# hammershock/3dgs-avatar-release

Measured on AMD Instinct MI355X. Metric: render fps (fwd+bwd) @200k Gaussians 1024x1024 SH3, higher is better.
Workload: dtype f32; 1 GPU; config3: 200k Gaussians, 1024x1024, SH deg 3, forward+backward; shs+scales+rotations inputs, L1 loss (L1 fused into the rasterizer: l1_target); tile_rect=1, l1=fused, long_lists=0, gaussians=200000, width=1024, height=1024, sh_degree=3, frames_per_rank=1857, total_frames=1857, ranks=1, backend=none, parallelism=frames sharded x1

## Files before the change

3dgs-avatar-release_amd/csrc/binning.hip:

```cpp
#include "common.h"

__global__ __launch_bounds__(256) void first_pair_kernel(const uint32_t* __restrict__ tiles,
                                                         const uint32_t* __restrict__ wave_tiles, float* __restrict__ rec,
                                                         int P, unsigned long long* __restrict__ count,
                                                         unsigned long long* host_count) {
    __shared__ unsigned long long wb[4];
    const int tid = threadIdx.x, lane = tid & 63, wid = tid >> 6;
    const int w0 = 4 * (int)blockIdx.x;
    unsigned long long before = 0;
    for (int w = tid; w < w0; w += 256) before += wave_tiles[w];
#pragma unroll
    for (int d = 32; d >= 1; d >>= 1) before += __shfl_xor(before, d, 64);
    if (lane == 0) wb[wid] = before;
    const int i = blockIdx.x * 256 + tid;
    const uint32_t v = i < P ? tiles[i] : 0u;
    uint32_t x = v;
#pragma unroll
    for (int d = 1; d < 64; d <<= 1) {
        const uint32_t y = __shfl_up(x, d, 64);
        if (lane >= d) x += y;
    }
    __syncthreads();
    const unsigned long long block_base = (wb[0] + wb[1]) + (wb[2] + wb[3]);
    uint32_t woff = 0;
// ... 395 lines not shown
                                                          const uint32_t* __restrict__ keys, int mode, int ntiles,
                                                          uint32_t* __restrict__ order, const PairCount pc,
                                                          const FillJob fill, const LongLists ll) {
    if (blockIdx.x > 0) {
        if (fill.clean && *fill.clean == MARKS_CLEAN) return;
        const uint4 ones = make_uint4(0xFFFFFFFFu, 0xFFFFFFFFu, 0xFFFFFFFFu, 0xFFFFFFFFu);
        for (size_t k = (size_t)(blockIdx.x - 1) * 1024 + threadIdx.x; k < fill.quads; k += (size_t)(gridDim.x - 1) * 1024)
            if (fill.stream) store_stream(&fill.ptr[k], ones); else fill.ptr[k] = ones;
        return;
    }
    __shared__ uint32_t hist[1024];
    __shared__ uint32_t wmax[16];
    __shared__ uint32_t wsum[16];
    if (mode < 0) return;
    tile_order_body<HELD>(ranges, keys, mode, ntiles, order, pc, ll, hist, wmax, wsum);
}

#define BM_LD 33
#ifndef TW_STOP_AFTER
#define TW_STOP_AFTER 99
#endif
template <bool CW>
__global__ __launch_bounds__(TBK_THREADS) void tile_write_kernel(const uint4* __restrict__ ranklist,
                                                                 const uint32_t* __restrict__ seg_start, int P, int gx,
                                                                 int gy, int nbx, int nblocks, int nseg, int ntiles,
                                                                 const uint32_t* __restrict__ seg_cnt,
                                                                 const uint32_t* __restrict__ tile_tot,
                                                                 uint2* __restrict__ ranges, uint32_t* __restrict__ order,
                                                                 uint32_t* __restrict__ point_list, const PairCount pc,
                                                                 const LongLists ll) {
// ... 197 lines not shown

int launch_tile_order(const uint32_t* ranges, const uint32_t* keys, int mode, int ntiles, uint32_t* order, PairCount pc,
                      FillJob fill, LongLists ll, int debug, hipStream_t s) {
    const size_t pieces = (fill.quads + 1023) / 1024;
    const int side = fill.ptr ? (int)(pieces < 255 ? pieces : 255) : 0;
    if (ntiles <= 32 * 1024)
        hipLaunchKernelGGL(tile_order_kernel<true>, dim3(1 + side), dim3(1024), 0, s, reinterpret_cast<const uint2*>(ranges),
                           keys, mode, ntiles, order, pc, fill, ll);
    else
        hipLaunchKernelGGL(tile_order_kernel<false>, dim3(1 + side), dim3(1024), 0, s, reinterpret_cast<const uint2*>(ranges),
                           keys, mode, ntiles, order, pc, fill, ll);
    GS_LAUNCH_CHECK("tile_order", debug, s);
    return GS_OK;
}

int launch_tile_lists(const uint4* ranklist, const uint32_t* chunk_pairs, uint32_t* seg_start, int P, int gx, int gy, TileCounts tc, uint32_t* ranges,
                      uint32_t* order, uint32_t* point_list, PairCount pc, LongLists ll, bool totals_zeroed, int debug,
                      hipStream_t s) {
    uint32_t* seg_cnt = tc.seg_cnt;
    const BinGrid G = bin_grid(gx, gy);
    const int nseg = bin_segments(G, P);
    const int ntiles = gx * gy;
    if (!totals_zeroed) {
        const int zrc = gs_zero_async(tc.tile_tot, tc.zero_bytes, "tile_totals.zero", s);
        if (zrc != GS_OK) return zrc;
    }
    {
        int band_rows = TC_CELLS / (gx + 1) - 1;
        if (band_rows < 1) return GS_E_TOO_LARGE;
        if (band_rows > gy) band_rows = gy;
// ... 21 lines not shown
```

3dgs-avatar-release_amd/csrc/capi.hip:

```cpp
#include "common.h"
#include "boundary.h"
#include "sorted_lists.h"
#include <string.h>
#include <stdlib.h>
#include <atomic>
#include <chrono>
#include <mutex>
#include <vector>

static thread_local int g_last_hip = 0;
static thread_local const char* g_last_stage = "";
void gs_set_error(int hip_err, const char* stage) {
    g_last_hip = hip_err;
    g_last_stage = stage;
}

struct TuneSwitch {
    const char* name;
    int key, def;
    const char* env;
    bool (*ok)(int);
};
static const TuneSwitch k_tune[GS_TUNE_COUNT] = {
    {"xcd_map", GS_TUNE_XCD_MAP, 1, nullptr, nullptr},
    {"depth_sort", GS_TUNE_DEPTH_SORT, 1, nullptr, nullptr},
    {"nt_stores", GS_TUNE_NT_STORES, 1, nullptr, nullptr},
    {"bwd_chunks", GS_TUNE_BWD_CHUNKS, 1, nullptr, nullptr},
    {"fwd4", GS_TUNE_FWD4, 1, "GSPLAT_FWD4", nullptr},
    {"small_tiles", GS_TUNE_SMALL_TILES, BWD_CHUNK_MAX_TILES, nullptr, nullptr},
    {"shared_qlist", GS_TUNE_SHARED_QLIST, 1, nullptr, nullptr},
    {"ones_fast", GS_TUNE_ONES_FAST, 1, nullptr, nullptr},
    {"bwd_order", GS_TUNE_BWD_ORDER, 1, nullptr, nullptr},
    {"fwd_marks", GS_TUNE_FWD_MARKS, 1, nullptr, nullptr},
    {"fwdc_ch", GS_TUNE_FWDC_CH, (int)FWDC_CH_MIN, "GSPLAT_FWDC_CH", [](int v) { return v >= 64 && (v & (v - 1)) == 0; }},
    {"fwdc_div", GS_TUNE_FWDC_DIV, (int)FWD4_TOTAL_DIV, "GSPLAT_FWDC_DIV", [](int v) { return v >= 1; }},
};
struct TuneState {
    std::atomic<int> v[GS_TUNE_COUNT];
    TuneState() {
        for (const TuneSwitch& t : k_tune) {
            int value = t.def;
            if (const char* e = t.env ? getenv(t.env) : nullptr) {
                const int x = atoi(e);
                if (!t.ok || t.ok(x)) value = x;
            }
            v[t.key].store(value);
        }
    }
};
static TuneState& tune_state() {
// ... 136 lines not shown
    ql.ckpt = ql.chunks > 1 ? writable(im.ckpt) : nullptr;
    ql.ck_start = ql.chunks > 1 ? writable(im.ck_start) : nullptr;
    return ql;
}
template <bool RO>
static void quad_lists_chunked(QuadLists& ql, const ImgView& own, const ImgViewT<RO>& list) {
    ql.chunked = 1;
    ql.cw_hdr = list.cw_hdr;
    ql.cw_units = list.cw_units;
    ql.cw_items = list.cw_items;
    ql.cw_q = own.cw_q;
    ql.cw_flag = own.cw_flag;
    ql.cw_done = own.cw_done;
    ql.cw_rec = own.cw_rec;
}
static int sync_if_debug(const GsFwdArgs* a, const char* stage, hipStream_t s) {
    if (!a->debug) return GS_OK;
    const hipError_t e = hipStreamSynchronize(s);
    if (e != hipSuccess) { gs_set_error((int)e, stage); return GS_E_HIP; }
    return GS_OK;
}

extern "C" {

int gs_xcc_probe(uint32_t* xcc, int32_t n_blocks, void* stream) {
    if (!xcc || n_blocks <= 0) return GS_E_BAD_ARG;
    hipStream_t s = (hipStream_t)stream;
    hipLaunchKernelGGL(xcc_probe_kernel, dim3((unsigned)n_blocks), dim3(64), 0, s, xcc);
    GS_LAUNCH_CHECK("xcc_probe", 0, s);
    return GS_OK;
// ... 118 lines not shown
        StageScope sc_("ranges_order", s);
        rc = launch_tile_order(im.ranges, nullptr, 0, im.ntiles, im.order, pc, FillJob{nullptr, 0},
                               LongLists{0, nullptr, im.cw_hdr, nullptr}, a->debug, s);
        if (rc != GS_OK) return rc;
    }
    QuadLists ql = quad_lists(im, b, a->long_lists);
    if (chunked) quad_lists_chunked(ql, im, im);
    if (cap > 0) {
        ql.marks = (gs_tune_get(GS_TUNE_FWD_MARKS) && !a->forward_only) ? b.marks : nullptr;
        ql.mark_quads = (size_t)cap;
        ql.marks_flag = b.marks_flag;
    }
    ql.l1_target = a->l1_target;
    ql.l1_part = im.l1_part;
    ql.l1_loss = a->l1_loss;
    { StageScope sc_("render_fwd", s);
    rc = launch_render_forward(g.rec, a->P > 0 ? b.point_list : nullptr, im.ranges, im.order, a->bg, a->W, a->H, out_color,
                               im.final_T, im.n_contrib, ql, s); }
    if (rc != GS_OK) return rc;
    return sync_if_debug(a, "render_forward", s);
}

int gs_forward_render(const GsFwdArgs* a, void* geom, size_t geom_bytes, void* binning, size_t binning_bytes,
                      void* img, size_t img_bytes, int64_t D, float* out_color, void* stream) {
    GS_CAPTURE_OK_IF(stream, a && !a->debug && a->frame_stats == nullptr);
    return forward_phase2(a, geom, geom_bytes, binning, binning_bytes, img, img_bytes, D, out_color, stream, false);
}

int gs_forward(const GsFwdArgs* a, void* geom, size_t geom_bytes, void* binning, size_t binning_bytes, int64_t capacity,
               void* img, size_t img_bytes, int32_t* radii, int64_t* count_host_pinned, float* out_color,
               int64_t* num_rendered, void* stream) {
    if (!count_host_pinned || !num_rendered || capacity < 0) return GS_E_BAD_ARG;
    GS_NO_CAPTURE(stream);
    volatile int64_t* word = count_host_pinned;
// ... 95 lines not shown
    const ImgViewRO im = img_state(img, a->W, a->H, a->long_lists);
    if (img_bytes < im.total) return GS_E_WORKSPACE;
    return launch_opacity_image(im.final_T, a->bg, a->W, a->H, opacity, (hipStream_t)stream);
}

static int backward_impl(const GsFwdArgs* a, const int32_t* radii, const void* geom, size_t geom_bytes, void* binning,
                         size_t binning_bytes, const void* img, size_t img_bytes, int64_t D, const float* out_color,
                         const float* dL_dpix, const float* dL_dopacity_img, void* scratch, size_t scratch_bytes,
                         const GsGrads* gr, void* stream, const GsSecondImage* second = nullptr) {
    GS_CAPTURE_OK_IF(stream, a && !a->debug);
    GeomViewRO g;
    BinView b;
    ImgViewRO im;
    int rc = frame_states(a, geom, geom_bytes, binning, binning_bytes, img, img_bytes, D, &g, &b, &im, [&]() -> int {
        if (!out_color || (!dL_dpix && !a->l1_target) || !gr || (a->P > 0 && !scratch)) return GS_E_BAD_ARG;
        if (a->P > 0 && (!radii || !gr->dL_dmeans3D || !gr->dL_dmeans2D || !gr->dL_dcolors || !gr->dL_dopacity || !gr->dL_dcov3D))
            return GS_E_BAD_ARG;
        if (a->P > 0 && a->shs && !gr->dL_dsh) return GS_E_BAD_ARG;
        if (a->P > 0 && a->scales && (!gr->dL_dscales || !gr->dL_drotations)) return GS_E_BAD_ARG;
        if (!aligned(gr->dL_drotations, 16)) return GS_E_BAD_ARG;
        return GS_OK;
    });
    if (rc != GS_OK) return rc;
    if (a->P > 0 && scratch_bytes < scratch_total_bytes(D, a->P, im.ntiles)) return GS_E_WORKSPACE;
    if (a->P == 0) return GS_OK;
    hipStream_t s = (hipStream_t)stream;
    float* const sums = (float*)((char*)scratch + scratch_rows_bytes(D));
    if (D > 0) {
        const QuadLists ql = quad_lists(im, b, a->long_lists);
        SecondImage si{nullptr, nullptr, nullptr, nullptr, nullptr};
        if (second) {
            const ImgViewRO im2 = img_state(second->img, a->W, a->H, second->long_lists);
            if (second->img_bytes < im2.total || im2.bwd_chunks != im.bwd_chunks) return GS_E_BAD_ARG;
            si = SecondImage{second->colors, second->out_color, second->dL_dpix, ql.chunks > 1 ? im2.ckpt : nullptr, im2.all_ones};
        }
        uint32_t* const q8 = reinterpret_cast<uint32_t*>(b.marks);
        uint32_t* const own_order = (uint32_t*)((char*)sums + scratch_sums_bytes(a->P));
        const bool order_here = gs_tune_get(GS_TUNE_BWD_ORDER) != 0;
        { StageScope sc_("tile_order", s);
        rc = launch_tile_order(im.ranges, ql.qcount, order_here ? 1 : -1, im.ntiles, own_order, PairCount{nullptr, 0},
                               FillJob{b.marks, (size_t)D, gs_tune_get(GS_TUNE_NT_STORES) & 1, b.marks_flag},
                               LongLists{0, nullptr}, a->debug, s); }
        if (rc != GS_OK) return rc;
        { StageScope sc_("render_bwd", s);
        rc = launch_render_backward(g.rec, im.ranges, order_here ? own_order : im.order, a->W, a->H, ql, out_color, dL_dpix,
                                    dL_dopacity_img, im.final_T, a->bg, (float*)scratch, q8, second ? &si : nullptr,
                                    L1Grad{a->l1_target, a->l1_grad}, s); }
        if (rc != GS_OK) return rc;
        rc = sync_if_debug(a, "render_backward", s);
        if (rc != GS_OK) return rc;
    }
    { StageScope sc_("gaussian_bwd", s);
    rc = launch_gaussian_backward(*a, radii, g.rec, g.tiles, g.clamped, reinterpret_cast<const uint32_t*>(b.marks),
                                  (const float*)scratch, sums, b.marks_flag, *gr, s); }
    if (rc != GS_OK || !second || !second->dL_dcolors) return rc;
    { StageScope sc_("second_colors", s);
    rc = launch_second_colors(g.rec, g.tiles, radii, b.point_list, im.ranges, im.order, im.n_contrib, second->dL_dpix, a->P, a->W,
                              a->H, D, PairCount{g.count + COUNT_PAIRS, (uint32_t)D}, few_long_lists_mode(im.ntiles, a->long_lists),
                              scratch, scratch_rows_bytes(D),
                              second->dL_dcolors, a->debug, s); }
// ... 172 lines not shown
```

3dgs-avatar-release_amd/csrc/common.h:

```cpp
#pragma once
#include <hip/hip_runtime.h>
#include <stdint.h>
#include <stddef.h>
#include <type_traits>
#include "../../include/gsplat_mi355.h"
#include "ordered_sum.h"

#define TILE 16
#define WAVE 64
#define REC_F 12
#define GS_MAX_PAIRS 0x3FFFFFFFll

static inline size_t align_up(size_t x, size_t a) { return (x + a - 1) / a * a; }
struct Carver {
    char* base;
    size_t o = 0;
    explicit Carver(void* b) : base(static_cast<char*>(b)) {}
    template <class T>
    T* take(size_t count) {
        const size_t at = o;
        o = align_up(o + count * sizeof(T), 256);
        return base ? reinterpret_cast<T*>(base + at) : nullptr;
    }
};
// ... 90 lines not shown
    G.nby = (gy + TB_H - 1) / TB_H;
    G.nblocks = G.nbx * G.nby;
#ifndef TB_TARGET_WGS
#define TB_TARGET_WGS 512
#endif
    int s = (TB_TARGET_WGS + G.nblocks - 1) / G.nblocks;
    G.nseg_max = s < 1 ? 1 : (s > TB_MAX_SEG ? TB_MAX_SEG : s);
    return G;
}
static inline int bin_segments(const BinGrid& G, int P) {
    int s = (P + 1023) / 1024;
    if (s < 1) s = 1;
    return s < G.nseg_max ? s : G.nseg_max;
}

enum { GS_TUNE_XCD_MAP = 0, GS_TUNE_DEPTH_SORT = 1, GS_TUNE_NT_STORES = 2, GS_TUNE_BWD_CHUNKS = 3, GS_TUNE_FWD4 = 4, GS_TUNE_SMALL_TILES = 5, GS_TUNE_SHARED_QLIST = 6, GS_TUNE_ONES_FAST = 7, GS_TUNE_BWD_ORDER = 8, GS_TUNE_FWD_MARKS = 9, GS_TUNE_FWDC_CH = 10, GS_TUNE_FWDC_DIV = 11, GS_TUNE_COUNT = 12 };
int gs_tune_get(int key);

#define BWD_CH 128
#define BWD_KMAX 16
#define BWD_CHUNK_MAX_TILES 2048
#define FWD4_MAX_TILES 2048
#define FWD4_MIN_LIST 512u
#ifndef FWD4_TOTAL_DIV
#define FWD4_TOTAL_DIV 320ull
#endif

#define FWDC_CH_MIN 256u
#define FWDC_SPARSE_PAIRS 524288ull
#define FWDC_MAX_UNITS 4096
#define FWDC_MAX_TILES (FWDC_MAX_UNITS / 2)
#define FWDC_Q_WORDS (8 * FWDC_MAX_UNITS * 4)
#define FWDC_Q_BYTES ((size_t)FWDC_Q_WORDS * 4 + 64)
#ifdef FWDC_PROF
#define FWDC_SLOTS 9
#else
#define FWDC_SLOTS 8
#endif
#define FWDC_DEAD 0x80000000u
#define FWDC_SPIN_MAX (1 << 16)
struct ImgLayout {
    size_t ranges, n_contrib, final_T, ncon_c, tile_nmax, order, seg_cnt, tile_tot, all_ones, cw_flag, cw_done, cw_q, tile_zero_bytes, l1_part, ckpt, ck_start, cw_hdr, cw_units, cw_items, cw_rec, total;
    int gx, gy, bwd_chunks;
};
static inline bool few_long_lists_mode(int ntiles, int long_lists) {
    return ntiles <= gs_tune_get(GS_TUNE_SMALL_TILES) || long_lists != 0;
}
static inline ImgLayout img_layout(int W, int H, int long_lists = 0) {
    ImgLayout L;
    size_t o = 0;
    auto take = [&](size_t bytes) { size_t at = o; o = align_up(o + bytes, 256); return at; };
    L.gx = (W + TILE - 1) / TILE;
    L.gy = (H + TILE - 1) / TILE;
    const size_t nt = (size_t)L.gx * L.gy;
    L.ranges = take(nt * 8);
    L.n_contrib = take((size_t)W * H * 4);
    L.final_T = take((size_t)W * H * 4);
// ... 12 lines not shown
        L.cw_done = take(nt * 16);
        L.cw_q = take(FWDC_Q_BYTES);
        L.tile_zero_bytes = L.cw_q + FWDC_Q_BYTES - L.tile_tot;
    }
    L.l1_part = take(nt * 16);
    L.bwd_chunks = fl ? BWD_KMAX : 1;
    L.ckpt = take(nt * 4 * (size_t)(L.bwd_chunks - 1) * 64 * 16);
    L.ck_start = take(nt * 4 * (size_t)L.bwd_chunks * 4);
    L.cw_hdr = L.cw_units = L.cw_items = L.cw_rec = 0;
    if (cw) {
        L.cw_hdr = take(64);
        L.cw_units = take((size_t)FWDC_MAX_UNITS * 8);
        L.cw_items = take((size_t)FWDC_Q_WORDS * 4);
        L.cw_rec = take((size_t)FWDC_MAX_UNITS * 4 * FWDC_SLOTS * 64 * 4);
    }
    L.total = o;
    return L;
}

template <bool RO>
struct StateCarve {
    typename std::conditional<RO, const char, char>::type* base;
    StateCarve(typename std::conditional<RO, const void, void>::type* state) : base(static_cast<decltype(base)>(state)) {}
    template <class T>
    void operator()(T*& field, size_t offset, bool present = true) const {
        field = (base && present) ? reinterpret_cast<T*>(base + offset) : nullptr;
    }
};
template <bool RO>
struct GeomViewT {
// ... 17 lines not shown
    size_t total;
};
template <bool RO>
struct ImgViewT {
    template <class T> using ptr = typename std::conditional<RO, const T, T>::type*;
    ptr<uint32_t> ranges, n_contrib;
    ptr<float> final_T;
    ptr<uint32_t> ncon_c, qcount , order, seg_cnt, tile_tot, all_ones;
    ptr<uint32_t> cw_flag, cw_done, cw_q, cw_xcc_mask ;
    ptr<float> l1_part;
    ptr<float4> ckpt;
    ptr<uint32_t> ck_start, cw_hdr;
    ptr<uint2> cw_units;
    ptr<uint32_t> cw_items;
    ptr<float> cw_rec;
    size_t tile_zero_bytes;
    int cw_clear_words;
    size_t total;
    int gx, gy, ntiles, bwd_chunks;
};
typedef GeomViewT<false> GeomView;
typedef GeomViewT<true> GeomViewRO;
typedef BinViewT<false> BinView;
typedef BinViewT<true> BinViewRO;
typedef ImgViewT<false> ImgView;
typedef ImgViewT<true> ImgViewRO;

template <class Void >
static inline GeomViewT<std::is_const<Void>::value> geom_state(Void* base, int P) {
    constexpr bool RO = std::is_const<Void>::value;
// ... 22 lines not shown
}
template <class Void >
static inline ImgViewT<std::is_const<Void>::value> img_state(Void* base, int W, int H, int long_lists) {
    constexpr bool RO = std::is_const<Void>::value;
    const ImgLayout L = img_layout(W, H, long_lists);
    const StateCarve<RO> at{base};
    const bool cw = L.cw_rec != 0;
    ImgViewT<RO> v;
    at(v.ranges, L.ranges); at(v.n_contrib, L.n_contrib); at(v.final_T, L.final_T); at(v.ncon_c, L.ncon_c);
    at(v.qcount, L.tile_nmax); at(v.order, L.order); at(v.seg_cnt, L.seg_cnt); at(v.tile_tot, L.tile_tot);
    at(v.all_ones, L.all_ones);
    at(v.cw_flag, L.cw_flag, cw); at(v.cw_done, L.cw_done, cw); at(v.cw_q, L.cw_q, cw);
    at(v.cw_xcc_mask, L.cw_q + (size_t)FWDC_Q_WORDS * 4, cw);
    at(v.l1_part, L.l1_part); at(v.ckpt, L.ckpt); at(v.ck_start, L.ck_start);
    at(v.cw_hdr, L.cw_hdr, cw); at(v.cw_units, L.cw_units, cw); at(v.cw_items, L.cw_items, cw); at(v.cw_rec, L.cw_rec, cw);
    v.tile_zero_bytes = L.tile_zero_bytes;
    v.cw_clear_words = cw ? (int)((L.cw_q + FWDC_Q_BYTES - L.cw_flag) / 4) : 0;
    v.total = L.total; v.gx = L.gx; v.gy = L.gy; v.ntiles = L.gx * L.gy; v.bwd_chunks = L.bwd_chunks;
    return v;
}
static inline unsigned long long* not_ones_word(const GeomViewRO& first) {
    return const_cast<unsigned long long*>(first.count) + COUNT_NOT_ONES;
}

static inline int radix_passes(int bits) { return (bits + 7) / 8; }

void gs_set_error(int hip_err, const char* stage);
#define GS_LAUNCH_CHECK(stage, dbg, stream)                                            \
    do {                                                                               \
        hipError_t e__ = hipGetLastError();                                            \
// ... 152 lines not shown


int launch_first_pair(const uint32_t* tiles, const uint32_t* wave_tiles, float* rec, unsigned long long* count,
                      unsigned long long* host_count, int P, int debug, hipStream_t s);
int launch_rank_list(const uint32_t* sorted_idx, const float* rec, const uint32_t* tiles, uint4* ranklist,
                     uint32_t* chunk_pairs, int P, int debug, hipStream_t s);
struct TileCounts { uint32_t *seg_cnt, *tile_tot; size_t zero_bytes; uint32_t* xcc_mask = nullptr; };
struct LongLists { int mark; long long* stats; uint32_t* cw_hdr = nullptr; uint2* cw_units = nullptr; uint32_t ch_min = FWDC_CH_MIN;
                   uint32_t* cw_items = nullptr; const uint32_t* xcc_mask = nullptr;
                   uint32_t total_div = (uint32_t)FWD4_TOTAL_DIV; };
int launch_tile_lists(const uint4* ranklist, const uint32_t* chunk_pairs, uint32_t* seg_start, int P, int gx, int gy, TileCounts tc, uint32_t* ranges,
                      uint32_t* order, uint32_t* point_list, PairCount pc, LongLists ll, bool totals_zeroed, int debug,
                      hipStream_t s);

int launch_loss_final(const float* partial, int nparts, float inv_n, float* loss, hipStream_t s);

#define MARKS_CLEAN 0x600DF111u
struct FillJob { uint4* ptr; size_t quads; int stream = 0; const uint32_t* clean = nullptr;  };

typedef uint32_t gs_u32x4 __attribute__((ext_vector_type(4)));
__device__ __forceinline__ void store_stream(uint4* p, uint4 v) {
    gs_u32x4 x = {v.x, v.y, v.z, v.w};
    __builtin_nontemporal_store(x, reinterpret_cast<gs_u32x4*>(p));
}
int launch_tile_order(const uint32_t* ranges, const uint32_t* keys, int mode, int ntiles, uint32_t* order, PairCount pc,
                      FillJob fill, LongLists ll, int debug, hipStream_t s);
struct QuadLists {
    uint32_t* qlist;
    uint32_t* ncon_c;
    uint32_t* qcount;
// ... 10 lines not shown
    const float* src_cw_rec = nullptr;
    const float* src_final_T = nullptr;
    const uint32_t* src_qcount = nullptr;
    const uint32_t* src_n_contrib = nullptr;
    const unsigned long long* not_ones = nullptr;
    float4* ckpt = nullptr;
    uint32_t* ck_start = nullptr;
    int chunks = 1;
    uint4* marks = nullptr;
    size_t mark_quads = 0;
    uint32_t* marks_flag = nullptr;
    uint32_t* all_ones = nullptr;
    const float* l1_target = nullptr;
    float* l1_part = nullptr;
    float* l1_loss = nullptr;
};
int launch_render_forward(const float* rec, const uint32_t* point_list, const uint32_t* ranges, const uint32_t* order,
                          const float* bg, int W, int H, float* out_color, float* final_T, uint32_t* n_contrib,
                          const QuadLists& ql, hipStream_t s);
struct SecondImage {
    const float* colors;
    const float* out_color;
    const float* dL_dpix;
    const float4* ckpt;
    const uint32_t* all_ones;
};
struct L1Grad { const float* target; const float* grad; };
int launch_render_backward(const float* rec, const uint32_t* ranges, const uint32_t* order, int W, int H,
                           const QuadLists& ql, const float* out_color, const float* dL_dpix, const float* dL_dopa,
                           const float* final_T, const float* bg, float* qrows, uint32_t* q8, const SecondImage* second,
// ... 23 lines not shown
```

3dgs-avatar-release_amd/csrc/gaussian_bwd.hip:

```cpp
#include "common.h"
#include "gs_math.h"
#include "blend.h"

#ifndef GB_THREADS
#define GB_THREADS 256
#endif

__global__ __launch_bounds__(256) void segment_reduce_kernel(int P, const int32_t* __restrict__ radii,
                                                             const float4* __restrict__ rec,
                                                             const uint32_t* __restrict__ tiles,
                                                             const uint32_t* __restrict__ q8,
                                                             const float4* __restrict__ qrows,
                                                             float4* __restrict__ sums, uint32_t* __restrict__ marks_flag) {
    const int t = blockIdx.x * blockDim.x + threadIdx.x;
    if (t == 0 && marks_flag) *marks_flag = 0u;
    const int i = t >> 4, j = t & 15;
    const int rs = j >> 1, h = j & 1;
    float a0 = 0.f, a1 = 0.f, a2 = 0.f, a3 = 0.f, a8 = 0.f;
    const bool in = i < P;
    float4 r0 = make_float4(0.f, 0.f, 0.f, 0.f), r1 = r0;
    if (in && radii[i] > 0) {
        const uint32_t off = __float_as_uint(rec[(size_t)i * 3 + 2].y);
        const uint32_t nrows = 4u * tiles[i];
        if (j < 2) {
// ... 40 lines not shown
    }
    if (in && j < 2) {
        const float A2 = (-0.5f * LOG2E_F) * r0.z, B2 = -LOG2E_F * r0.w, C2 = (-0.5f * LOG2E_F) * r1.x, op = r1.y;
        const float il2 = 1.0f / LOG2E_F;
        if (j == 0) {
            const float oa0 = op * f[0], oa1 = op * f[1];
            sums[(size_t)i * 3] = make_float4((2.f * A2 * oa0 + B2 * oa1) * il2, (2.f * C2 * oa1 + B2 * oa0) * il2,
                                              f[2] * (-0.5f * op), f[3] * (-0.5f * op));
            sums[(size_t)i * 3 + 2] = make_float4(f[4], 0.f, 0.f, 0.f);
        } else {
            sums[(size_t)i * 3 + 1] = make_float4(f[0] * (-0.5f * op), f[1], f[2], f[3]);
        }
    }
}

template <bool antialiasing>
__global__ __launch_bounds__(256) void gaussian_bwd_kernel(
    int P, int deg, int M, const float* __restrict__ means3D, const float* __restrict__ scales, float scale_modifier,
    const float* __restrict__ rotations, const float* __restrict__ shs, const float* __restrict__ cov3D_precomp,
    const float* __restrict__ viewmatrix, const float* __restrict__ projmatrix, const float* __restrict__ campos, int W,
    int H, float tanfovx, float tanfovy, float fx, float fy, const int32_t* __restrict__ radii,
    const uint32_t* __restrict__ clamped, const float4* __restrict__ sums, float* __restrict__ dL_dmeans3D, float* __restrict__ dL_dmeans2D,
    float* __restrict__ dL_dsh, float* __restrict__ dL_dcolors, float* __restrict__ dL_dopacity,
    float* __restrict__ dL_dscales, float* __restrict__ dL_drotations, float* __restrict__ dL_dcov3D,
    const float4* __restrict__ rec) {
    extern __shared__ float sh_tile[];
    const int i = blockIdx.x * blockDim.x + threadIdx.x;
    const int ld = sh_tile_ld(M);
    const int row0 = blockIdx.x * blockDim.x;
    const int nrows = min((int)blockDim.x, P - row0);
    if (shs) {
// ... 8 lines not shown
    {
        const float4 a0 = sums[(size_t)i * 3], a1 = sums[(size_t)i * 3 + 1];
        const float a2 = sums[(size_t)i * 3 + 2].x;
        s[0] = a0.x; s[1] = a0.y; s[2] = a0.z; s[3] = a0.w;
        s[4] = a1.x; s[5] = a1.y; s[6] = a1.z; s[7] = a1.w;
        s[8] = a2;
    }
    const float g2x = s[0] * (0.5f * W), g2y = s[1] * (0.5f * H);
    const float gA = s[2], gB = s[3], gC = s[4], gO = s[5];
    const float gR[3] = {s[6], s[7], s[8]};

    dL_dmeans2D[3 * i] = g2x;
    dL_dmeans2D[3 * i + 1] = g2y;
    dL_dmeans2D[3 * i + 2] = 0.f;
    dL_dopacity[i] = gO;
    dL_dcolors[3 * i] = gR[0];
    dL_dcolors[3 * i + 1] = gR[1];
    dL_dcolors[3 * i + 2] = gR[2];

    float gm[3] = {0.f, 0.f, 0.f};
    float gc[6] = {0.f, 0.f, 0.f, 0.f, 0.f, 0.f};
    float gs[3] = {0.f, 0.f, 0.f};
    float gq[4] = {0.f, 0.f, 0.f, 0.f};

    if (live) {
        float V[16], PV[16];
#pragma unroll
        for (int k = 0; k < 16; k++) { V[k] = viewmatrix[k]; PV[k] = projmatrix[k]; }
        const float3 mean = make_float3(means3D[3 * i], means3D[3 * i + 1], means3D[3 * i + 2]);
        float c6[6];
        float3 sc = make_float3(0, 0, 0);
        float4 q = make_float4(1, 0, 0, 0);
        if (cov3D_precomp) {
// ... 154 lines not shown
                for (int r_ = 0; r_ < 3; r_++) dR[r_][c_] = dL[r_][c_] * sv[c_];
            }
            const float r = q.x, x = q.y, y = q.z, z = q.w;
            gq[0] = 2 * z * (dR[1][0] - dR[0][1]) + 2 * y * (dR[0][2] - dR[2][0]) + 2 * x * (dR[2][1] - dR[1][2]);
            gq[1] = 2 * y * (dR[0][1] + dR[1][0]) + 2 * z * (dR[0][2] + dR[2][0]) + 2 * r * (dR[2][1] - dR[1][2]) - 4 * x * (dR[2][2] + dR[1][1]);
            gq[2] = 2 * x * (dR[0][1] + dR[1][0]) + 2 * r * (dR[0][2] - dR[2][0]) + 2 * z * (dR[2][1] + dR[1][2]) - 4 * y * (dR[2][2] + dR[0][0]);
            gq[3] = 2 * r * (dR[1][0] - dR[0][1]) + 2 * x * (dR[0][2] + dR[2][0]) + 2 * y * (dR[2][1] + dR[1][2]) - 4 * z * (dR[1][1] + dR[0][0]);
        }
    } else if (shs) {
        float* gsh = sh_tile + threadIdx.x * ld;
        for (int k = 0; k < M * 3; k++) gsh[k] = 0.f;
    }
    dL_dmeans3D[3 * i] = gm[0];
    dL_dmeans3D[3 * i + 1] = gm[1];
    dL_dmeans3D[3 * i + 2] = gm[2];
#pragma unroll
    for (int k = 0; k < 6; k++) dL_dcov3D[6 * i + k] = gc[k];
    if (dL_dscales) {
        dL_dscales[3 * i] = gs[0];
        dL_dscales[3 * i + 1] = gs[1];
        dL_dscales[3 * i + 2] = gs[2];
    }
    if (dL_drotations) reinterpret_cast<float4*>(dL_drotations)[i] = make_float4(gq[0], gq[1], gq[2], gq[3]);
    }
    if (shs) {
        __syncthreads();
        sh_tile_store(dL_dsh + (size_t)row0 * M * 3, sh_tile, nrows, M * 3, ld);
    }
}

int launch_gaussian_backward(const GsFwdArgs& a, const int32_t* radii, const float* rec, const uint32_t* tiles,
                             const uint32_t* clamped, const uint32_t* q8, const float* qrows, float* sums,
                             uint32_t* marks_flag, const GsGrads& g, hipStream_t s) {
    const float fy = a.H / (2.0f * a.tanfovy), fx = a.W / (2.0f * a.tanfovx);
    hipLaunchKernelGGL(segment_reduce_kernel, dim3((unsigned)(((size_t)a.P * 16 + 255) / 256)), dim3(256), 0, s, a.P, radii,
                       reinterpret_cast<const float4*>(rec), tiles, q8,
                       reinterpret_cast<const float4*>(qrows), reinterpret_cast<float4*>(sums), marks_flag);
    GS_LAUNCH_CHECK("segment_reduce", a.debug, s);
    const size_t lds = a.shs ? (size_t)GB_THREADS * ((3 * a.M) | 1) * sizeof(float) : 0;
    hipLaunchKernelGGL(a.antialiasing ? gaussian_bwd_kernel<true> : gaussian_bwd_kernel<false>,
                       dim3((a.P + GB_THREADS - 1) / GB_THREADS), dim3(GB_THREADS), lds, s, a.P, a.sh_degree, a.M, a.means3D,
                       a.scales, a.scale_modifier, a.rotations, a.shs, a.cov3D_precomp, a.viewmatrix, a.projmatrix,
                       a.campos, a.W, a.H, a.tanfovx, a.tanfovy, fx, fy, radii, clamped,
                       reinterpret_cast<const float4*>(sums), g.dL_dmeans3D, g.dL_dmeans2D,
                       g.dL_dsh, g.dL_dcolors, g.dL_dopacity, g.dL_dscales, g.dL_drotations, g.dL_dcov3D,
                       reinterpret_cast<const float4*>(rec));
    GS_LAUNCH_CHECK("gaussian_backward", a.debug, s);
    return GS_OK;
}
```

3dgs-avatar-release_amd/csrc/ordered_sum.h:

```cpp
#pragma once
#include <hip/hip_runtime.h>
#include <stdint.h>
#include <stddef.h>
#include <type_traits>

struct ZeroJob { uint32_t* ptr; int words; };
__device__ __forceinline__ void zero_job(const ZeroJob z) {
    for (int k = blockIdx.x * blockDim.x + threadIdx.x; k < z.words; k += gridDim.x * blockDim.x) z.ptr[k] = 0u;
}

template <int CTRL, int ROW_MASK>
__device__ __forceinline__ uint32_t dpp_or_zero(uint32_t v) {
    return (uint32_t)__builtin_amdgcn_update_dpp(0, (int)v, CTRL, ROW_MASK, 0xF, false);
}
__device__ __forceinline__ uint32_t wave_scan_incl(uint32_t x) {
    x += dpp_or_zero<0x111, 0xF>(x);
    x += dpp_or_zero<0x112, 0xF>(x);
    x += dpp_or_zero<0x114, 0xF>(x);
    x += dpp_or_zero<0x118, 0xF>(x);
    x += dpp_or_zero<0x142, 0xA>(x);
    x += dpp_or_zero<0x143, 0xC>(x);
    return x;
}
__device__ __forceinline__ uint32_t row_scan_incl(uint32_t x) {
// ... 57 lines not shown
}
template <int T>
__device__ __forceinline__ float strided_sum(const float* __restrict__ p, int n) {
    float acc = 0.0f;
    for (int i = threadIdx.x; i < n; i += T) acc += p[i];
    return acc;
}
template <int T, class Order, bool SCALED>
__global__ __launch_bounds__(T) void ordered_final_kernel(const float* __restrict__ partial, int nb, float scale,
                                                          float* __restrict__ out) {
    __shared__ float ws[T / 64];
    const float s = block_sum<T, Order>(strided_sum<T>(partial + (size_t)blockIdx.x * nb, nb), ws);
    if (threadIdx.x == 0) out[blockIdx.x] = SCALED ? s * scale : s;
}

__device__ __forceinline__ double runs64_sum(const double* __restrict__ p, int nb, double* run) {
    const int l = threadIdx.x;
    const int per = (nb + 63) / 64, b0 = min(nb, l * per), b1 = min(nb, b0 + per);
    double a = 0.0;
    for (int b = b0; b < b1; b++) a += p[b];
    run[l] = a;
    __syncthreads();
    double s = 0.0;
    if (l == 0)
        for (int k = 0; k < 64; k++) s += run[k];
    return s;
}
```

3dgs-avatar-release_amd/csrc/render_fwd.hip:

```cpp
#include "common.h"
#include "blend.h"
#include <type_traits>

struct FwdArgs {
    const float4* __restrict__ rec;
    const uint32_t* __restrict__ point_list;
    const uint2* __restrict__ ranges;
    const uint32_t* __restrict__ order;
    const float* __restrict__ bg;
    int W, H, gx, ntiles, xmap;
    float* __restrict__ out_color;
    float* __restrict__ final_T;
    uint32_t* __restrict__ n_contrib;
    uint32_t* __restrict__ qlist;
    uint32_t* __restrict__ ncon_c;
    uint32_t* __restrict__ qcount;
    float4* __restrict__ ckpt;
    uint32_t* __restrict__ ck_start;
    int chunks;
    const uint32_t* __restrict__ src_qcount;
    const uint32_t* __restrict__ src_n_contrib;
    const unsigned long long* __restrict__ not_ones;
    uint4* __restrict__ marks;
    size_t mark_quads;
// ... 875 lines not shown
    const dim3 grid(render_grid_blocks(gx * gy, xmap) + A.cw_blocks);
    const bool fq = ql.src_qcount != nullptr;
    if (ql.four_waves) {
        if (fq) hipLaunchKernelGGL(render_fwd_small_kernel<true>, grid, dim3(FWD4_BATCH), 0, s, A);
        else hipLaunchKernelGGL(render_fwd_small_kernel<false>, grid, dim3(FWD4_BATCH), 0, s, A);
    } else {
        if (A.cw_blocks) {
            if (fq) hipLaunchKernelGGL(render_fwd_cw_kernel<true>, grid, dim3(64), 0, s, A);
            else hipLaunchKernelGGL(render_fwd_cw_kernel<false>, grid, dim3(64), 0, s, A);
        } else {
            if (fq) hipLaunchKernelGGL(render_fwd_kernel<true>, grid, dim3(64), 0, s, A);
            else hipLaunchKernelGGL(render_fwd_kernel<false>, grid, dim3(64), 0, s, A);
        }
    }
    GS_LAUNCH_CHECK("render_forward", 0, s);
    if (ql.l1_target)
        return launch_loss_final(ql.l1_part, gx * gy * 4, 1.0f / (3.0f * (float)W * (float)H), ql.l1_loss, s);
    return GS_OK;
}

__global__ __launch_bounds__(256) void opacity_image_kernel(const float* __restrict__ final_T, const float* __restrict__ bg,
                                                            int n, float* __restrict__ out) {
    const int i = blockIdx.x * blockDim.x + threadIdx.x;
    if (i >= n) return;
    const float Tf = final_T[i];
    out[i] = (1.0f - Tf) + Tf * bg[0];
}

int launch_opacity_image(const float* final_T, const float* bg, int W, int H, float* out, hipStream_t s) {
    const int n = W * H;
    hipLaunchKernelGGL(opacity_image_kernel, dim3((n + 255) / 256), dim3(256), 0, s, final_T, bg, n, out);
    GS_LAUNCH_CHECK("opacity_image", 0, s);
// ... 3 lines not shown
```

3dgs-avatar-release_amd/diff_gaussian_rasterization/__init__.py:

```python
import ctypes
import os
import sys
import threading
import weakref
from typing import NamedTuple

import torch
import torch.nn as nn

from gsplat_mi355 import _lib

__all__ = ["GaussianRasterizationSettings", "GaussianRasterizer", "rasterize_gaussians"]


class GaussianRasterizationSettings(NamedTuple):
    image_height: int
    image_width: int
    tanfovx: float
    tanfovy: float
    bg: torch.Tensor
    scale_modifier: float
    viewmatrix: torch.Tensor
    projmatrix: torch.Tensor
    sh_degree: int
# ... 501 lines not shown
                _keep = []
                a = _make_args(settings, means3D, sh if has_sh else None, colors_precomp if has_col else None, opacities,
                               scales if has_sr else None, rotations if has_sr else None,
                               cov3Ds_precomp if has_cov else None, _keep, long_lists=fr.long_lists)
            a.l1_target = ctx.l1_target.data_ptr() if use_l1 else None
            a.l1_loss = None
            a.l1_grad = g_l1.data_ptr() if use_l1 else None
            gp = g.data_ptr() if g is not None else None
            sptr = _lib.stream_ptr(dev)
            scratch_bytes = _size("gs_backward_scratch_bytes", D, P, W, H)
            scratch = torch.empty(scratch_bytes, dtype=torch.uint8, device=dev)
            M = int(sh.shape[1]) if has_sh else 0
            f = dict(dtype=torch.float32, device=dev)
            d_means3D = torch.empty(P, 3, **f)
            d_means2D = torch.empty(P, 3, **f)
            d_colors = torch.empty(P, 3, **f)
            d_opacity = torch.empty(P, 1, **f)
            d_cov3D = torch.empty(P, 6, **f)
            d_sh = torch.empty(P, M, 3, **f) if has_sh else None
            d_scales = torch.empty(P, 3, **f) if has_sr else None
            d_rot = torch.empty(P, 4, **f) if has_sr else None
            gr = _lib.GsGrads(_lib.ptr(d_means3D), _lib.ptr(d_means2D), _lib.ptr(d_sh), _lib.ptr(d_colors),
                              _lib.ptr(d_opacity), _lib.ptr(d_scales), _lib.ptr(d_rot), _lib.ptr(d_cov3D))
            lead = (ctypes.byref(a), radii.data_ptr(), geom.data_ptr(), geom.numel(), binning.data_ptr(), binning.numel(),
                    img.data_ptr(), img.numel(), D, color.data_ptr(), gp)
            tail = (scratch.data_ptr(), scratch_bytes, ctypes.byref(gr), sptr)
            si = None
            if g_inv is not None:
                colors2, color2, img2 = ctx.saved_tensors[12:15]
                g2 = torch.zeros(3, H, W, **f)
                g2[0].copy_(g_inv.reshape(H, W))
                d_colors2 = torch.empty(P, 3, **f)
                si = _lib.GsSecondImage(colors2.data_ptr(), color2.data_ptr(), g2.data_ptr(), img2.data_ptr(), img2.numel(),
# ... 3 lines not shown
                                        second["img"].data_ptr(), second["img"].numel(), int(second["long_lists"]))
            if si is not None:
                fn, mid = L.gs_backward_with_second, (ctypes.byref(si),)
            elif g_op is None:
                fn, mid = L.gs_backward, ()
            else:
                fn, mid = L.gs_backward_with_opacity, (g_op.data_ptr(),)
            _lib.check(fn(*lead, *mid, *tail))
            if g_inv is not None:
                hook = getattr(sys.modules.get("gsplat_mi355.debug"), "second_colors_hook", None)
                if hook is not None:
                    hook(d_colors2)
                invz = colors2[:, 0]
                view = _f32c(settings.viewmatrix.to(dev), "viewmatrix")
                d_means3D.addcmul_((d_colors2.sum(1) * invz * invz).unsqueeze(1), view[:3, 2].unsqueeze(0), value=-1.0)
        return (d_means3D, d_means2D, d_sh, d_colors if has_col else None, d_opacity, d_scales, d_rot,
                d_cov3D if has_cov else None, None, None, None, None, None)


class GaussianRasterizer(nn.Module):
    def __init__(self, raster_settings):
        super().__init__()
        self.raster_settings = raster_settings

    def markVisible(self, positions):
        L = _lib.load()
        rs = self.raster_settings
        with torch.no_grad():
            pos = _f32c(positions, "positions")
            P = int(pos.shape[0])
            out = torch.zeros(P, dtype=torch.uint8, device=pos.device)
            view = _f32c(rs.viewmatrix.to(pos.device), "viewmatrix")
# ... 28 lines not shown
```

Baseline: 1782 frames/s.

## Compute backward tile order during forward loss reduction; skip unused gradient writes

```diff
diff --git a/3dgs-avatar-release_amd/csrc/binning.hip b/3dgs-avatar-release_amd/csrc/binning.hip
--- a/3dgs-avatar-release_amd/csrc/binning.hip
+++ b/3dgs-avatar-release_amd/csrc/binning.hip
@@ -433,6 +433,20 @@
     __shared__ uint32_t wsum[16];
     if (mode < 0) return;
     tile_order_body<HELD>(ranges, keys, mode, ntiles, order, pc, ll, hist, wmax, wsum);
+}
+
+template <bool HELD>
+__global__ __launch_bounds__(1024) void loss_final_order_kernel(const float* __restrict__ partial, int nparts, float inv_n,
+                                                                float* __restrict__ loss, const uint32_t* __restrict__ qcount,
+                                                                int ntiles, uint32_t* __restrict__ order) {
+    __shared__ uint32_t hist[1024];
+    __shared__ uint32_t wmax[16];
+    __shared__ uint32_t wsum[16];
+    if (blockIdx.x == 0) {
+        wide_final_sum(partial, nparts, inv_n, loss, reinterpret_cast<float*>(wsum));
+        return;
+    }
+    tile_order_body<HELD>(nullptr, qcount, 1, ntiles, order, PairCount{nullptr, 0}, LongLists{0, nullptr}, hist, wmax, wsum);
 }
 
 #define BM_LD 33
@@ -660,6 +674,16 @@
     return GS_OK;
 }
 
+int launch_loss_final_with_order(const float* partial, int nparts, float inv_n, float* loss, const uint32_t* qcount, int ntiles,
+                                 uint32_t* order, hipStream_t s) {
+    if (ntiles <= 32 * 1024)
+        hipLaunchKernelGGL(loss_final_order_kernel<true>, dim3(2), dim3(1024), 0, s, partial, nparts, inv_n, loss, qcount, ntiles, order);
+    else
+        hipLaunchKernelGGL(loss_final_order_kernel<false>, dim3(2), dim3(1024), 0, s, partial, nparts, inv_n, loss, qcount, ntiles, order);
+    GS_LAUNCH_CHECK("loss_final_order", 0, s);
+    return GS_OK;
+}
+
 int launch_tile_lists(const uint4* ranklist, const uint32_t* chunk_pairs, uint32_t* seg_start, int P, int gx, int gy, TileCounts tc, uint32_t* ranges,
                       uint32_t* order, uint32_t* point_list, PairCount pc, LongLists ll, bool totals_zeroed, int debug,
                       hipStream_t s) {
diff --git a/3dgs-avatar-release_amd/csrc/capi.hip b/3dgs-avatar-release_amd/csrc/capi.hip
--- a/3dgs-avatar-release_amd/csrc/capi.hip
+++ b/3dgs-avatar-release_amd/csrc/capi.hip
@@ -34,6 +34,7 @@
     {"fwd_marks", GS_TUNE_FWD_MARKS, 1, nullptr, nullptr},
     {"fwdc_ch", GS_TUNE_FWDC_CH, (int)FWDC_CH_MIN, "GSPLAT_FWDC_CH", [](int v) { return v >= 64 && (v & (v - 1)) == 0; }},
     {"fwdc_div", GS_TUNE_FWDC_DIV, (int)FWD4_TOTAL_DIV, "GSPLAT_FWDC_DIV", [](int v) { return v >= 1; }},
+    {"order_with_sum", GS_TUNE_ORDER_WITH_SUM, 1, nullptr, nullptr},
 };
 struct TuneState {
     std::atomic<int> v[GS_TUNE_COUNT];
@@ -200,6 +201,33 @@
     ql.cw_done = own.cw_done;
     ql.cw_rec = own.cw_rec;
 }
+struct OrderNote { const void* binning; const void* img; int64_t D; int ntiles; void* stream; };
+#define ORDER_NOTES 8
+static OrderNote g_order_notes[ORDER_NOTES];
+static unsigned g_order_next = 0;
+static std::mutex g_order_mu;
+static void order_note_forward(const void* binning, const void* img, int64_t D, int ntiles, void* stream, bool valid) {
+    std::lock_guard<std::mutex> lk(g_order_mu);
+    for (OrderNote& n : g_order_notes)
+        if (n.binning && (n.binning == binning || n.img == img)) n = OrderNote{nullptr, nullptr, 0, 0, nullptr};
+    if (!valid || !binning) return;
+    OrderNote* slot = nullptr;
+    for (OrderNote& n : g_order_notes)
+        if (!n.binning) { slot = &n; break; }
+    if (!slot) slot = &g_order_notes[g_order_next++ % ORDER_NOTES];
+    *slot = OrderNote{binning, img, D, ntiles, stream};
+}
+static bool order_note_take(const void* binning, const void* img, int64_t D, int ntiles, void* stream) {
+    std::lock_guard<std::mutex> lk(g_order_mu);
+    bool hit = false;
+    for (OrderNote& n : g_order_notes) {
+        if (!n.binning || n.binning != binning) continue;
+        hit = n.img == img && n.D == D && n.ntiles == ntiles && n.stream == stream;
+        n = OrderNote{nullptr, nullptr, 0, 0, nullptr};
+    }
+    return hit;
+}
+
 static int sync_if_debug(const GsFwdArgs* a, const char* stage, hipStream_t s) {
     if (!a->debug) return GS_OK;
     const hipError_t e = hipStreamSynchronize(s);
@@ -348,10 +376,15 @@
     ql.l1_target = a->l1_target;
     ql.l1_part = im.l1_part;
     ql.l1_loss = a->l1_loss;
+    const bool order_job = a->l1_target && ql.marks && a->P > 0 && gs_tune_get(GS_TUNE_BWD_ORDER) &&
+                           gs_tune_get(GS_TUNE_ORDER_WITH_SUM) && !stream_is_capturing(stream);
+    if (order_job) ql.bwd_order = im.bwd_order;
+    order_note_forward(binning, img, cap, im.ntiles, stream, false);
     { StageScope sc_("render_fwd", s);
     rc = launch_render_forward(g.rec, a->P > 0 ? b.point_list : nullptr, im.ranges, im.order, a->bg, a->W, a->H, out_color,
                                im.final_T, im.n_contrib, ql, s); }
     if (rc != GS_OK) return rc;
+    if (order_job) order_note_forward(binning, img, cap, im.ntiles, stream, true);
     return sync_if_debug(a, "render_forward", s);
 }
 
@@ -477,8 +510,8 @@
     ImgViewRO im;
     int rc = frame_states(a, geom, geom_bytes, binning, binning_bytes, img, img_bytes, D, &g, &b, &im, [&]() -> int {
         if (!out_color || (!dL_dpix && !a->l1_target) || !gr || (a->P > 0 && !scratch)) return GS_E_BAD_ARG;
-        if (a->P > 0 && (!radii || !gr->dL_dmeans3D || !gr->dL_dmeans2D || !gr->dL_dcolors || !gr->dL_dopacity || !gr->dL_dcov3D))
-            return GS_E_BAD_ARG;
+        if (a->P > 0 && (!radii || !gr->dL_dmeans3D || !gr->dL_dmeans2D || !gr->dL_dopacity)) return GS_E_BAD_ARG;
+        if (a->P > 0 && ((a->colors_precomp && !gr->dL_dcolors) || (a->cov3D_precomp && !gr->dL_dcov3D))) return GS_E_BAD_ARG;
         if (a->P > 0 && a->shs && !gr->dL_dsh) return GS_E_BAD_ARG;
         if (a->P > 0 && a->scales && (!gr->dL_dscales || !gr->dL_drotations)) return GS_E_BAD_ARG;
         if (!aligned(gr->dL_drotations, 16)) return GS_E_BAD_ARG;
@@ -500,13 +533,17 @@
         uint32_t* const q8 = reinterpret_cast<uint32_t*>(b.marks);
         uint32_t* const own_order = (uint32_t*)((char*)sums + scratch_sums_bytes(a->P));
         const bool order_here = gs_tune_get(GS_TUNE_BWD_ORDER) != 0;
-        { StageScope sc_("tile_order", s);
-        rc = launch_tile_order(im.ranges, ql.qcount, order_here ? 1 : -1, im.ntiles, own_order, PairCount{nullptr, 0},
-                               FillJob{b.marks, (size_t)D, gs_tune_get(GS_TUNE_NT_STORES) & 1, b.marks_flag},
-                               LongLists{0, nullptr}, a->debug, s); }
+        const bool noted = order_note_take(binning, img, D, im.ntiles, stream);
+        const bool order_ready = noted && order_here && gs_tune_get(GS_TUNE_ORDER_WITH_SUM) && !stream_is_capturing(stream);
+        if (!order_ready) {
+            StageScope sc_("tile_order", s);
+            rc = launch_tile_order(im.ranges, ql.qcount, order_here ? 1 : -1, im.ntiles, own_order, PairCount{nullptr, 0},
+                                   FillJob{b.marks, (size_t)D, gs_tune_get(GS_TUNE_NT_STORES) & 1, b.marks_flag},
+                                   LongLists{0, nullptr}, a->debug, s);
+        }
         if (rc != GS_OK) return rc;
         { StageScope sc_("render_bwd", s);
-        rc = launch_render_backward(g.rec, im.ranges, order_here ? own_order : im.order, a->W, a->H, ql, out_color, dL_dpix,
+        rc = launch_render_backward(g.rec, im.ranges, order_ready ? im.bwd_order : (order_here ? own_order : im.order), a->W, a->H, ql, out_color, dL_dpix,
                                     dL_dopacity_img, im.final_T, a->bg, (float*)scratch, q8, second ? &si : nullptr,
                                     L1Grad{a->l1_target, a->l1_grad}, s); }
         if (rc != GS_OK) return rc;
diff --git a/3dgs-avatar-release_amd/csrc/common.h b/3dgs-avatar-release_amd/csrc/common.h
--- a/3dgs-avatar-release_amd/csrc/common.h
+++ b/3dgs-avatar-release_amd/csrc/common.h
@@ -128,7 +128,7 @@
     return s < G.nseg_max ? s : G.nseg_max;
 }
 
-enum { GS_TUNE_XCD_MAP = 0, GS_TUNE_DEPTH_SORT = 1, GS_TUNE_NT_STORES = 2, GS_TUNE_BWD_CHUNKS = 3, GS_TUNE_FWD4 = 4, GS_TUNE_SMALL_TILES = 5, GS_TUNE_SHARED_QLIST = 6, GS_TUNE_ONES_FAST = 7, GS_TUNE_BWD_ORDER = 8, GS_TUNE_FWD_MARKS = 9, GS_TUNE_FWDC_CH = 10, GS_TUNE_FWDC_DIV = 11, GS_TUNE_COUNT = 12 };
+enum { GS_TUNE_XCD_MAP = 0, GS_TUNE_DEPTH_SORT = 1, GS_TUNE_NT_STORES = 2, GS_TUNE_BWD_CHUNKS = 3, GS_TUNE_FWD4 = 4, GS_TUNE_SMALL_TILES = 5, GS_TUNE_SHARED_QLIST = 6, GS_TUNE_ONES_FAST = 7, GS_TUNE_BWD_ORDER = 8, GS_TUNE_FWD_MARKS = 9, GS_TUNE_FWDC_CH = 10, GS_TUNE_FWDC_DIV = 11, GS_TUNE_ORDER_WITH_SUM = 12, GS_TUNE_COUNT = 13 };
 int gs_tune_get(int key);
 
 #define BWD_CH 128
@@ -154,7 +154,7 @@
 #define FWDC_DEAD 0x80000000u
 #define FWDC_SPIN_MAX (1 << 16)
 struct ImgLayout {
-    size_t ranges, n_contrib, final_T, ncon_c, tile_nmax, order, seg_cnt, tile_tot, all_ones, cw_flag, cw_done, cw_q, tile_zero_bytes, l1_part, ckpt, ck_start, cw_hdr, cw_units, cw_items, cw_rec, total;
+    size_t ranges, n_contrib, final_T, ncon_c, tile_nmax, order, seg_cnt, tile_tot, all_ones, cw_flag, cw_done, cw_q, tile_zero_bytes, l1_part, ckpt, ck_start, cw_hdr, cw_units, cw_items, cw_rec, bwd_order, total;
     int gx, gy, bwd_chunks;
 };
 static inline bool few_long_lists_mode(int ntiles, int long_lists) {
@@ -197,6 +197,7 @@
         L.cw_items = take((size_t)FWDC_Q_WORDS * 4);
         L.cw_rec = take((size_t)FWDC_MAX_UNITS * 4 * FWDC_SLOTS * 64 * 4);
     }
+    L.bwd_order = take(nt * 4);
     L.total = o;
     return L;
 }
@@ -244,6 +245,7 @@
     ptr<uint2> cw_units;
     ptr<uint32_t> cw_items;
     ptr<float> cw_rec;
+    ptr<uint32_t> bwd_order;
     size_t tile_zero_bytes;
     int cw_clear_words;
     size_t total;
@@ -296,6 +298,7 @@
     at(v.cw_xcc_mask, L.cw_q + (size_t)FWDC_Q_WORDS * 4, cw);
     at(v.l1_part, L.l1_part); at(v.ckpt, L.ckpt); at(v.ck_start, L.ck_start);
     at(v.cw_hdr, L.cw_hdr, cw); at(v.cw_units, L.cw_units, cw); at(v.cw_items, L.cw_items, cw); at(v.cw_rec, L.cw_rec, cw);
+    at(v.bwd_order, L.bwd_order);
     v.tile_zero_bytes = L.tile_zero_bytes;
     v.cw_clear_words = cw ? (int)((L.cw_q + FWDC_Q_BYTES - L.cw_flag) / 4) : 0;
     v.total = L.total; v.gx = L.gx; v.gy = L.gy; v.ntiles = L.gx * L.gy; v.bwd_chunks = L.bwd_chunks;
@@ -478,6 +481,8 @@
                       hipStream_t s);
 
 int launch_loss_final(const float* partial, int nparts, float inv_n, float* loss, hipStream_t s);
+int launch_loss_final_with_order(const float* partial, int nparts, float inv_n, float* loss, const uint32_t* qcount, int ntiles,
+                                 uint32_t* order, hipStream_t s);
 
 #define MARKS_CLEAN 0x600DF111u
 struct FillJob { uint4* ptr; size_t quads; int stream = 0; const uint32_t* clean = nullptr;  };
@@ -518,6 +523,7 @@
     const float* l1_target = nullptr;
     float* l1_part = nullptr;
     float* l1_loss = nullptr;
+    uint32_t* bwd_order = nullptr;
 };
 int launch_render_forward(const float* rec, const uint32_t* point_list, const uint32_t* ranges, const uint32_t* order,
                           const float* bg, int W, int H, float* out_color, float* final_T, uint32_t* n_contrib,
diff --git a/3dgs-avatar-release_amd/csrc/gaussian_bwd.hip b/3dgs-avatar-release_amd/csrc/gaussian_bwd.hip
--- a/3dgs-avatar-release_amd/csrc/gaussian_bwd.hip
+++ b/3dgs-avatar-release_amd/csrc/gaussian_bwd.hip
@@ -78,7 +78,7 @@
     }
 }
 
-template <bool antialiasing>
+template <bool antialiasing, bool WCOL, bool WCOV>
 __global__ __launch_bounds__(256) void gaussian_bwd_kernel(
     int P, int deg, int M, const float* __restrict__ means3D, const float* __restrict__ scales, float scale_modifier,
     const float* __restrict__ rotations, const float* __restrict__ shs, const float* __restrict__ cov3D_precomp,
@@ -117,9 +117,11 @@
     dL_dmeans2D[3 * i + 1] = g2y;
     dL_dmeans2D[3 * i + 2] = 0.f;
     dL_dopacity[i] = gO;
-    dL_dcolors[3 * i] = gR[0];
-    dL_dcolors[3 * i + 1] = gR[1];
-    dL_dcolors[3 * i + 2] = gR[2];
+    if (WCOL) {
+        dL_dcolors[3 * i] = gR[0];
+        dL_dcolors[3 * i + 1] = gR[1];
+        dL_dcolors[3 * i + 2] = gR[2];
+    }
 
     float gm[3] = {0.f, 0.f, 0.f};
     float gc[6] = {0.f, 0.f, 0.f, 0.f, 0.f, 0.f};
@@ -304,8 +306,10 @@
     dL_dmeans3D[3 * i] = gm[0];
     dL_dmeans3D[3 * i + 1] = gm[1];
     dL_dmeans3D[3 * i + 2] = gm[2];
-#pragma unroll
-    for (int k = 0; k < 6; k++) dL_dcov3D[6 * i + k] = gc[k];
+    if (WCOV || dL_dcov3D) {
+#pragma unroll
+        for (int k = 0; k < 6; k++) dL_dcov3D[6 * i + k] = gc[k];
+    }
     if (dL_dscales) {
         dL_dscales[3 * i] = gs[0];
         dL_dscales[3 * i + 1] = gs[1];
@@ -328,7 +332,20 @@
                        reinterpret_cast<const float4*>(qrows), reinterpret_cast<float4*>(sums), marks_flag);
     GS_LAUNCH_CHECK("segment_reduce", a.debug, s);
     const size_t lds = a.shs ? (size_t)GB_THREADS * ((3 * a.M) | 1) * sizeof(float) : 0;
-    hipLaunchKernelGGL(a.antialiasing ? gaussian_bwd_kernel<true> : gaussian_bwd_kernel<false>,
+    const auto kernel = [&]() {
+        const int k = (a.antialiasing ? 4 : 0) | (g.dL_dcolors ? 2 : 0) | (g.dL_dcov3D ? 1 : 0);
+        switch (k) {
+            case 0: return gaussian_bwd_kernel<false, false, false>;
+            case 1: return gaussian_bwd_kernel<false, false, true>;
+            case 2: return gaussian_bwd_kernel<false, true, false>;
+            case 3: return gaussian_bwd_kernel<false, true, true>;
+            case 4: return gaussian_bwd_kernel<true, false, false>;
+            case 5: return gaussian_bwd_kernel<true, false, true>;
+            case 6: return gaussian_bwd_kernel<true, true, false>;
+            default: return gaussian_bwd_kernel<true, true, true>;
+        }
+    }();
+    hipLaunchKernelGGL(kernel,
                        dim3((a.P + GB_THREADS - 1) / GB_THREADS), dim3(GB_THREADS), lds, s, a.P, a.sh_degree, a.M, a.means3D,
                        a.scales, a.scale_modifier, a.rotations, a.shs, a.cov3D_precomp, a.viewmatrix, a.projmatrix,
                        a.campos, a.W, a.H, a.tanfovx, a.tanfovy, fx, fy, radii, clamped,
diff --git a/3dgs-avatar-release_amd/csrc/ordered_sum.h b/3dgs-avatar-release_amd/csrc/ordered_sum.h
--- a/3dgs-avatar-release_amd/csrc/ordered_sum.h
+++ b/3dgs-avatar-release_amd/csrc/ordered_sum.h
@@ -95,6 +95,27 @@
     if (threadIdx.x == 0) out[blockIdx.x] = SCALED ? s * scale : s;
 }
 
+__device__ __forceinline__ void wide_final_sum(const float* __restrict__ partial, int nparts, float inv_n,
+                                               float* __restrict__ loss, float* ws) {
+    const int tid = threadIdx.x, lane = tid & 63, wid = tid >> 6;
+    float acc = 0.f;
+    for (int i0 = tid; i0 < nparts; i0 += 8 * 1024) {
+        float v[8];
+#pragma unroll
+        for (int u = 0; u < 8; u++) v[u] = (i0 + u * 1024 < nparts) ? partial[i0 + u * 1024] : 0.f;
+#pragma unroll
+        for (int u = 0; u < 8; u++) acc += v[u];
+    }
+    acc = wave_sum(acc);
+    if (lane == 0) ws[wid] = acc;
+    __syncthreads();
+    if (tid == 0) {
+        float t = 0.f;
+        for (int w = 0; w < 16; w++) t += ws[w];
+        loss[0] = t * inv_n;
+    }
+}
+
 __device__ __forceinline__ double runs64_sum(const double* __restrict__ p, int nb, double* run) {
     const int l = threadIdx.x;
     const int per = (nb + 63) / 64, b0 = min(nb, l * per), b1 = min(nb, b0 + per);
diff --git a/3dgs-avatar-release_amd/csrc/render_fwd.hip b/3dgs-avatar-release_amd/csrc/render_fwd.hip
--- a/3dgs-avatar-release_amd/csrc/render_fwd.hip
+++ b/3dgs-avatar-release_amd/csrc/render_fwd.hip
@@ -913,8 +913,11 @@
         }
     }
     GS_LAUNCH_CHECK("render_forward", 0, s);
-    if (ql.l1_target)
-        return launch_loss_final(ql.l1_part, gx * gy * 4, 1.0f / (3.0f * (float)W * (float)H), ql.l1_loss, s);
+    if (ql.l1_target) {
+        const float inv_n = 1.0f / (3.0f * (float)W * (float)H);
+        if (ql.bwd_order) return launch_loss_final_with_order(ql.l1_part, gx * gy * 4, inv_n, ql.l1_loss, ql.qcount, gx * gy, ql.bwd_order, s);
+        return launch_loss_final(ql.l1_part, gx * gy * 4, inv_n, ql.l1_loss, s);
+    }
     return GS_OK;
 }
 
diff --git a/3dgs-avatar-release_amd/diff_gaussian_rasterization/__init__.py b/3dgs-avatar-release_amd/diff_gaussian_rasterization/__init__.py
--- a/3dgs-avatar-release_amd/diff_gaussian_rasterization/__init__.py
+++ b/3dgs-avatar-release_amd/diff_gaussian_rasterization/__init__.py
@@ -539,9 +539,9 @@
             f = dict(dtype=torch.float32, device=dev)
             d_means3D = torch.empty(P, 3, **f)
             d_means2D = torch.empty(P, 3, **f)
-            d_colors = torch.empty(P, 3, **f)
+            d_colors = torch.empty(P, 3, **f) if has_col else None
             d_opacity = torch.empty(P, 1, **f)
-            d_cov3D = torch.empty(P, 6, **f)
+            d_cov3D = torch.empty(P, 6, **f) if has_cov else None
             d_sh = torch.empty(P, M, 3, **f) if has_sh else None
             d_scales = torch.empty(P, 3, **f) if has_sr else None
             d_rot = torch.empty(P, 4, **f) if has_sr else None
@@ -575,8 +575,7 @@
                 invz = colors2[:, 0]
                 view = _f32c(settings.viewmatrix.to(dev), "viewmatrix")
                 d_means3D.addcmul_((d_colors2.sum(1) * invz * invz).unsqueeze(1), view[:3, 2].unsqueeze(0), value=-1.0)
-        return (d_means3D, d_means2D, d_sh, d_colors if has_col else None, d_opacity, d_scales, d_rot,
-                d_cov3D if has_cov else None, None, None, None, None, None)
+        return (d_means3D, d_means2D, d_sh, d_colors, d_opacity, d_scales, d_rot, d_cov3D, None, None, None, None, None)
 
 
 class GaussianRasterizer(nn.Module):
```

After: 1799 frames/s, median of 6. No clear change (+1.0%).
